# jematy/SAHS-Deformable-Nerf

Measured on AMD Instinct MI355X. Metric: rendered rays/sec (coarse64+fine128, 8x256 MLP), higher is better.
Workload: dtype f32

## Files before the change

### sahs-deformable-nerf_amd/csrc/f32_pipe.hpp

```cpp
#pragma once
#include <hip/hip_runtime.h>
#include "sahs_common.hpp"
#include "sahs_layout.hpp"

namespace SAHS_NS {

constexpr int F32_THREADS = 512;
constexpr int F32_PTS_PER_WAVE = 16;
constexpr int F32_PTS_PER_WG = (F32_THREADS / WAVE) * F32_PTS_PER_WAVE;
constexpr int DBG_STRIDE = 56;
constexpr int LDS_BUF_FLOATS = CHUNK_FLOATS_MAX;
constexpr int LDS_BIAS_OFF = 2 * LDS_BUF_FLOATS;
constexpr int LDS_FLOATS = LDS_BIAS_OFF + ((BIAS_FLOATS + 3) / 4) * 4;
static_assert(LDS_FLOATS * 4 <= 160 * 1024, "LDS budget");

typedef __attribute__((address_space(3))) void *lds_ptr_t;
typedef const __attribute__((address_space(1))) void *gbl_ptr_t;
typedef const __attribute__((address_space(3))) float *lds_cfloat;
typedef const __attribute__((address_space(3))) f32x4 *lds_cf4;

constexpr int LDS_STASH_OFF = LDS_BIAS_OFF + ((BIAS_FLOATS + 3) / 4) * 4;
constexpr int STASH_FLOATS = 8;
constexpr int LDS_TOTAL_FLOATS = LDS_STASH_OFF + F32_PTS_PER_WG * STASH_FLOATS;
static_assert(LDS_TOTAL_FLOATS * 4 <= 160 * 1024, "LDS budget");
constexpr int PIECE_FLOATS = F32_THREADS * 4;
constexpr int MAX_PIECES = LDS_BUF_FLOATS / PIECE_FLOATS;
constexpr int A_AHEAD = 3;

struct Ctx {
    const float *stream;
    float *lds;
    int buf;
    int lane, q, wave;
    uint32_t off;
    uint32_t wrap_at, wrap_to;
    const f32x4 *nx_src; f32x4 *nx_dst;
    lds_cfloat bias_lane;

    __device__ __forceinline__ void begin_chunk(int next_floats)
    {
        if (off >= wrap_at) off = wrap_to;
        nx_src = reinterpret_cast<const f32x4 *>(stream + off) + lane;
        nx_dst = reinterpret_cast<f32x4 *>(lds + (buf ^ 1) * LDS_BUF_FLOATS);
        off += (uint32_t)next_floats;
    }
    __device__ __forceinline__ void issue_piece(int p)
    {
        const int base = p * F32_THREADS + wave * WAVE;
        __builtin_amdgcn_global_load_lds((gbl_ptr_t)(nx_src + base), (lds_ptr_t)(nx_dst + base), 16, 0, 0);
    }
    template <int N = 0>
    __device__ __forceinline__ void end_chunk()
    {
        if constexpr (N == 0) {
            __syncthreads();
        } else {
            asm volatile("s_waitcnt vmcnt(%0) lgkmcnt(0)\n\ts_barrier" ::"n"(N) : "memory");
        }
        buf ^= 1;
    }
    __device__ __forceinline__ const f32x4 *cur() const { return reinterpret_cast<const f32x4 *>(lds + buf * LDS_BUF_FLOATS); }
    __device__ __forceinline__ void refresh()
    {
        uint32_t a = (uint32_t)(uintptr_t)((__attribute__((address_space(3))) char *)lds) + (LDS_BIAS_OFF + 4 * q) * 4;
        asm volatile("" : "+v"(a));
        bias_lane = (lds_cfloat)(uintptr_t)a;
    }
    __device__ __forceinline__ f32x4 bias4(int off_) const { return *reinterpret_cast<lds_cf4>(bias_lane + off_); }
};

__device__ __forceinline__ f32x4 act4(f32x4 v, float slope)
{
    f32x4 o;
#pragma unroll
    for (int r = 0; r < 4; ++r) o[r] = fmaxf(v[r], v[r] * slope);
    return o;
}

constexpr int stores_behind_last_piece(int STEPS, int PAIR, int KB, int next_floats, int per_tile)
{
    const int npieces = (next_floats + PIECE_FLOATS - 1) / PIECE_FLOATS;
    const int pstep = (STEPS / 2 >= npieces) ? (STEPS / 2) / npieces : 1;
    if (per_tile == 0 || npieces > (STEPS + pstep - 1) / pstep) return 0;
    int n = 0;
    for (int s = (npieces - 1) * pstep; s < STEPS; ++s)
        if ((s % (PAIR * KB)) / PAIR == KB - 1) n += per_tile;
    return n > 48 ? 48 : n;
}

template <int KB0, int KB1, int NT, int NEXT, class EP>
__device__ __forceinline__ void dense_ep(Ctx &cx, const f32x4 *in0, const f32x4 *in1, f32x4 *out, EP &ep)
{
    constexpr int KB = KB0 + KB1;
    constexpr int G = pick_G(KB, NT);
    constexpr int NCH = NT / G;
    constexpr int PAIR = (G >= 2) ? 2 : 1;
    constexpr int STEPS = G * KB;
    constexpr int N_MID = stores_behind_last_piece(STEPS, PAIR, KB, G * KB * 256, EP::kStores), N_LAST = stores_behind_last_piece(STEPS, PAIR, KB, NEXT, EP::kStores);
#pragma unroll
    for (int c = 0; c < NCH; ++c) {
        const int nfl = (c + 1 < NCH) ? G * KB * 256 : NEXT;
        const int npieces = (nfl + PIECE_FLOATS - 1) / PIECE_FLOATS;
        const int pstep = (STEPS / 2 >= npieces) ? (STEPS / 2) / npieces : 1;
        cx.begin_chunk(nfl);
        const f32x4 *A = cx.cur() + cx.lane;
        auto frag = [&](int s) { const int pp = s / (PAIR * KB), r = s % (PAIR * KB); return ((pp * PAIR + r % PAIR) * KB + r / PAIR) * 64; };
        f32x4 a[A_AHEAD];
#pragma unroll
        for (int s = 0; s < A_AHEAD && s < STEPS; ++s) a[s] = A[frag(s)];
        f32x4 acc[PAIR];
#pragma unroll
        for (int s = 0; s < STEPS; ++s) {
            const int pp = s / (PAIR * KB), r = s % (PAIR * KB), m = r % PAIR, b = r / PAIR;
            const int t = c * G + pp * PAIR + m;
            if (b == 0) acc[m] = ep.first(cx, out, t);
            if (s % pstep == 0 && s / pstep < npieces) {
                cx.issue_piece(s / pstep);
                if (EP::kStores > 0 && s / pstep == npieces - 1) __builtin_amdgcn_sched_barrier(0);
            }
            const f32x4 x = (b < KB0) ? in0[b] : in1[b - KB0];
            const f32x4 w = a[s % A_AHEAD];
#pragma unroll
            for (int k = 0; k < 4; ++k) acc[m] = __builtin_amdgcn_mfma_f32_16x16x4f32(w[k], x[k], acc[m], 0, 0, 0);
            if (s + A_AHEAD < STEPS) a[s % A_AHEAD] = A[frag(s + A_AHEAD)];
            if (b == KB - 1) ep.template done<NT>(acc[m], out, t);
        }
#pragma unroll
        for (int pc = (STEPS + pstep - 1) / pstep; pc < MAX_PIECES; ++pc)
            if (pc < npieces) cx.issue_piece(pc);
        if (c + 1 < NCH) cx.template end_chunk<N_MID>();
        else cx.template end_chunk<N_LAST>();
    }
}

template <bool HAS_SAVE>
struct FwdEp {
    static constexpr int kStores = HAS_SAVE ? 1 : 0;
    int bias_off; bool accum; float slope;
    float *save;
    uint32_t *bsave;
    uint32_t sgn;
    __device__ __forceinline__ f32x4 first(const Ctx &cx, const f32x4 *out, int t) const { return accum ? out[t] : cx.bias4(bias_off + 16 * t); }
    template <int NT> __device__ __forceinline__ void done(const f32x4 &acc, f32x4 *out, int t)
    {
        f32x4 o = act4(acc, slope);
        asm volatile("" : "+v"(o));
        out[t] = o;
        if constexpr (HAS_SAVE) *reinterpret_cast<f32x4 *>(save + 16 * t) = o;
        if (bsave != nullptr) {
            uint32_t nib = 0u;
#pragma unroll
            for (int r = 0; r < 4; ++r) nib |= (o[r] > 0.0f) ? (1u << r) : 0u;
            if ((t & 1) == 0 && t + 1 < NT) sgn = nib;
            else reinterpret_cast<unsigned char *>(bsave)[t >> 1] = (unsigned char)((t & 1) ? (sgn | (nib << 4)) : nib);
        }
    }
};

template <int KB0, int KB1, int NT, int NEXT>
__device__ __forceinline__ void dense(Ctx &cx, const f32x4 *in0, const f32x4 *in1, f32x4 *out, int bias_off, bool accum, float slope)
{
    FwdEp<false> ep{bias_off, accum, slope, nullptr, nullptr, 0u};
    dense_ep<KB0, KB1, NT, NEXT>(cx, in0, in1, out, ep);
}
template <bool SAVING, int KB0, int KB1, int NT, int NEXT>
__device__ __forceinline__ void dense_sv(Ctx &cx, const f32x4 *in0, const f32x4 *in1, f32x4 *out, int bias_off, bool accum, float slope,
                                         float *save, uint32_t *bsave = nullptr)
{
    FwdEp<SAVING> ep{bias_off, accum, slope, save, SAVING ? bsave : nullptr, 0u};
    dense_ep<KB0, KB1, NT, NEXT>(cx, in0, in1, out, ep);
}

}
```

### sahs-deformable-nerf_amd/csrc/field_f32.hip

```cpp
#include <hip/hip_runtime.h>
#include "sahs_common.hpp"
#include "sahs_launchers.hpp"
#include "sahs_layout.hpp"
#include "f32_pipe.hpp"

namespace SAHS_NS {


struct RevArg { float p, lo; };
__device__ __forceinline__ RevArg rev_arg(float x)
{
    const float C_HI = 0.15915494f;
    const float C_LO = 6.4206382e-09f;
    RevArg r;
    r.p = x * C_HI;
    r.lo = fmaf(x, C_LO, fmaf(x, C_HI, -r.p));
    return r;
}
__device__ __forceinline__ float sin_octave(RevArg u, float scale, int fn)
{
    const float P = u.p * scale, Lo = u.lo * scale;
    const float f = (P - rintf(P)) + Lo;
    const float qf = rintf(4.0f * f);
    const float th = fmaf(qf, -0.25f, f) * 6.2831855f;
    const float z = th * th;
    const float sp = fmaf(th * z, fmaf(fmaf(-1.9515295891e-4f, z, 8.3321608736e-3f), z, -1.6666654611e-1f), th);
    const float cp = fmaf(z * z, fmaf(fmaf(2.443315711809948e-5f, z, -1.388731625493765e-3f), z, 4.166664568298827e-2f), fmaf(z, -0.5f, 1.0f));
    const int m = ((int)qf + fn) & 3;
    const float v = (m & 1) ? cp : sp;
    return (m & 2) ? -v : v;
}

template <int D, int L, int NB, int INC = 1>
__device__ __forceinline__ void pe_blocks(const float *v, int q, f32x4 *out)
{
    constexpr int D0 = INC ? D : 0;
    constexpr int W = D0 + 2 * D * L;
    const float v0 = v[0], v1 = v[D > 1 ? 1 : 0], v2 = v[D > 2 ? 2 : 0];
    const RevArg u0 = rev_arg(v0), u1 = rev_arg(v1), u2 = rev_arg(v2);
#pragma unroll
    for (int b = 0; b < NB; ++b)
#pragma unroll
        for (int r = 0; r < 4; ++r) {
            const int f = 16 * b + 4 * q + r;
            float val = 0.0f;
            if (f < D0) {
                val = (f == 0) ? v0 : ((f == 1) ? v1 : v2);
            } else if (f < W) {
                const int g = f - D0;
                const int k = g / (2 * D), rem = g % (2 * D);
                const int fn = rem / D, ax = rem % D;
                RevArg a;
                a.p = (ax == 0) ? u0.p : ((ax == 1) ? u1.p : u2.p);
                a.lo = (ax == 0) ? u0.lo : ((ax == 1) ? u1.lo : u2.lo);
                val = sin_octave(a, (float)(1 << k), fn);
            }
            out[b][r] = val;
        }
}

__device__ __forceinline__ void grid_blocks(const float *__restrict__ grid, float x, float y, float z, int q, f32x4 *out)
{
    const float R1 = (float)(G_RES - 1);
    const float ix = ((x + 1.0f) / 2.0f) * R1, iy = ((y + 1.0f) / 2.0f) * R1, iz = ((z + 1.0f) / 2.0f) * R1;
    const float fx = floorf(ix), fy = floorf(iy), fz = floorf(iz);
    const float x1 = fx + 1.0f, y1 = fy + 1.0f, z1 = fz + 1.0f;
    const float wx[2] = {x1 - ix, ix - fx}, wy[2] = {y1 - iy, iy - fy}, wz[2] = {z1 - iz, iz - fz};
    const bool ok = fx >= -1.0f && fx <= (float)G_RES && fy >= -1.0f && fy <= (float)G_RES && fz >= -1.0f && fz <= (float)G_RES;
    const int xi = ok ? (int)fx : -2, yi = ok ? (int)fy : -2, zi = ok ? (int)fz : -2;
    out[0] = f32x4{0.0f, 0.0f, 0.0f, 0.0f};
    out[1] = f32x4{0.0f, 0.0f, 0.0f, 0.0f};
#pragma unroll
    for (int n = 0; n < 8; ++n) {
        const int cx = xi + (n & 1), cy = yi + ((n >> 1) & 1), cz = zi + (n >> 2);
        const bool inb = cx >= 0 && cx < G_RES && cy >= 0 && cy < G_RES && cz >= 0 && cz < G_RES;
        const float wt = (wx[n & 1] * wy[(n >> 1) & 1]) * wz[n >> 2];
        const long vox = inb ? (((long)cz * G_RES + cy) * G_RES + cx) : 0;
        const f32x4 *g = reinterpret_cast<const f32x4 *>(grid + vox * D_GRID) + q;
        const f32x4 g0 = g[0], g1 = g[4];
        const float we = inb ? wt : 0.0f;
#pragma unroll
        for (int r = 0; r < 4; ++r) { out[0][r] = out[0][r] + g0[r] * we; out[1][r] = out[1][r] + g1[r] * we; }
    }
}

__device__ __forceinline__ void trunk_encodings(const float *stash, int q, f32x4 *enc)
{
    const float xw[3] = {stash[0], stash[1], stash[2]}, amb[2] = {stash[3], stash[4]};
    pe_blocks<3, L_XYZ, KB_XYZ>(xw, q, enc);
#if SAHS_MODEL != 2
    pe_blocks<AMB_DIM, L_AMB, KB_AMB, AMB_INC>(amb, q, enc + KB_XYZ);
#else
    (void)amb;
#endif
}

#define CHF(id) (kProg.layer[id].G * kProg.layer[id].KB * 256)

enum { FIELD_ALL = 0, FIELD_DEFORM = 1, FIELD_RADIANCE = 2, FIELD_ALL_FUSED = 6, FIELD_RADIANCE_FUSED = 7 };
constexpr int SPARSE_RING = 512;
static_assert(SPARSE_RING >= 255 + 128 && SPARSE_RING % 128 == 0, "a ring holds the carried count plus one tile");
__host__ __device__ constexpr long sparse_ring_slots(long tiles) { return tiles * F32_PTS_PER_WG < SPARSE_RING ? tiles * F32_PTS_PER_WG : SPARSE_RING; }
__host__ __device__ constexpr long sparse_ring_base(long ntiles, long grid, long g)
{
    const long tlo = ntiles / grid, rem = ntiles % grid;
    return g * sparse_ring_slots(tlo) + (g < rem ? g : rem) * (sparse_ring_slots(tlo + 1) - sparse_ring_slots(tlo));
}
constexpr int LDS_RING_FLOATS = 16;
struct SparseArgs {
    const float *noise;
    unsigned int *count;
    f32x4 *hdr;
    f32x4 *feat;
    unsigned int cap;
    int has_bg;
};
constexpr long SPARSE_HEAD_BYTES = 256, SPARSE_RECORD_BYTES = 16 + 16 * 16 * 4;
template <bool SAVE, int MODE>
__global__ void __launch_bounds__(F32_THREADS, 2)
field_forward_f32_kernel(const float *__restrict__ packed, const float *__restrict__ frame, int level, long P, int S,
                         const float *__restrict__ rays, int ray_stride, const float *__restrict__ zvals,
                         float *__restrict__ raw, float *__restrict__ dbg, float *__restrict__ actbuf,
                         float *__restrict__ xw, int xw_row, int xw_col0, const int *__restrict__ src, uint32_t *__restrict__ bits, SparseArgs sp)
{
#if SAHS_MODEL == 2
    static_assert(MODE == FIELD_ALL || MODE == FIELD_ALL_FUSED, "this model has no deformation nets to split off");
#endif
    constexpr bool FUSED = MODE == FIELD_ALL_FUSED || MODE == FIELD_RADIANCE_FUSED;
    constexpr bool XW_IN = MODE == FIELD_RADIANCE || MODE == FIELD_RADIANCE_FUSED;
    static_assert(!(SAVE && FUSED), "the sparse branches are an inference path");
    extern __shared__ __attribute__((aligned(16))) float lds[];
    Ctx cx;
    cx.stream = packed + PACK_STREAM_OFF + (long)level * STREAM_FLOATS;
    cx.lds = lds;
    cx.buf = 1;
    cx.lane = threadIdx.x & 63;
    cx.q = cx.lane >> 4;
    cx.wave = __builtin_amdgcn_readfirstlane(threadIdx.x >> 6);
    constexpr const Layer *Ly = kProg.layer;
    constexpr int L_START = XW_IN ? L_T0 : L_FIRST;
    cx.wrap_to = (uint32_t)Ly[L_START].stream_off;
    cx.wrap_at = (MODE == FIELD_DEFORM) ? (uint32_t)Ly[L_T0].stream_off : (FUSED ? (uint32_t)Ly[L_D0B].stream_off : (uint32_t)STREAM_FLOATS);
    cx.off = cx.wrap_to;
    const float *grid = packed + PACK_GRID_OFF;

    {
        const float *bsrc = frame + FRAME_BIAS_OFF + level * BIAS_FLOATS;
        for (int i = threadIdx.x; i < BIAS_FLOATS; i += F32_THREADS) lds[LDS_BIAS_OFF + i] = bsrc[i];
        cx.begin_chunk(CHF(L_START));
#pragma unroll
        for (int pc = 0; pc < (CHF(L_START) + PIECE_FLOATS - 1) / PIECE_FLOATS; ++pc) cx.issue_piece(pc);
        cx.end_chunk();
    }

    const long ntiles = (P + F32_PTS_PER_WG - 1) / F32_PTS_PER_WG;
    constexpr bool XW_AHEAD = MODE == FIELD_RADIANCE_FUSED;
    f32x4 nx_a = f32x4{0.0f, 0.0f, 0.0f, 0.0f};
    float nx_w1 = 0.0f;
    int nx_src = 0;
    uint32_t r_cnt = 0u, r_head = 0u, r_total = 0u, r_cap = 0u, r_base = 0u;
    uint32_t r_it = 0u, r_tiles = 0u;
    if constexpr (FUSED) {
        r_tiles = (uint32_t)__builtin_amdgcn_readfirstlane((int)(ntiles / gridDim.x + ((long)blockIdx.x < ntiles % gridDim.x ? 1 : 0)));
        r_cap = (uint32_t)sparse_ring_slots(r_tiles);
        r_base = (uint32_t)__builtin_amdgcn_readfirstlane((int)sparse_ring_base(ntiles, gridDim.x, blockIdx.x));
    }
    const uint32_t r_rows = FUSED ? (uint32_t)__builtin_amdgcn_readfirstlane((int)(ntiles / gridDim.x)) : 0u;
    auto fused_tile = [&](uint32_t k) -> long {
        const uint32_t col = k < r_rows ? (blockIdx.x + 61u * k) % gridDim.x : blockIdx.x;
        return (long)k * gridDim.x + col;
    };
    for (long tile_it = blockIdx.x; FUSED || tile_it < ntiles; tile_it += gridDim.x, ++r_it) {
        const long tile = FUSED ? fused_tile(r_it) : tile_it;
        bool has_tile = true, do_branch = false;
        uint32_t b_valid = 0u;
        if constexpr (FUSED) {
            has_tile = r_it < r_tiles;
            do_branch = has_tile ? r_cnt >= (uint32_t)F32_PTS_PER_WG : r_cnt > 0u;
            if (!has_tile && !do_branch) break;
            b_valid = r_cnt < (uint32_t)F32_PTS_PER_WG ? r_cnt : (uint32_t)F32_PTS_PER_WG;
            if (has_tile) {
                cx.wrap_at = do_branch ? (uint32_t)STREAM_FLOATS : (uint32_t)Ly[L_D0B].stream_off;
            } else {
                cx.off = (uint32_t)Ly[L_D0B].stream_off;
                cx.wrap_at = (uint32_t)STREAM_FLOATS;
                cx.begin_chunk(CHF(L_D0B));
#pragma unroll
                for (int pc = 0; pc < (CHF(L_D0B) + PIECE_FLOATS - 1) / PIECE_FLOATS; ++pc) cx.issue_piece(pc);
                cx.end_chunk();
            }
        }
        cx.refresh();
        int q_tile = cx.q;
        if constexpr (FUSED) { asm volatile("" : "+s"(cx.off)); asm volatile("" : "+v"(q_tile)); }
        const int q = q_tile;
        const long p_raw = tile * F32_PTS_PER_WG + cx.wave * F32_PTS_PER_WAVE + (cx.lane & 15);
        const long p = p_raw < P ? p_raw : P - 1;
        float *stash = lds + LDS_STASH_OFF + (cx.wave * F32_PTS_PER_WAVE + (cx.lane & 15)) * STASH_FLOATS;
        const bool dump = MODE == FIELD_ALL && dbg != nullptr && q == 0 && p_raw < P;
        float *dsl = dbg + p * DBG_STRIDE;
        const bool sv_on = SAVE && p_raw < P;
        long Psv = P;
        if constexpr (SAVE) asm volatile("" : "+s"(Psv));
#define SVP(c, w) (actbuf + (long)(c) * Psv + p * (long)(w) + 4 * q)
#define SV(c, w) SVP(c, w)
        const bool sb_on = sv_on && bits != nullptr;
        uint32_t *const bits_r = bits + (MODE == FIELD_ALL ? (long)sbits::BD_WORDS * Psv : 0L);
        const uint32_t sb_lane = (uint32_t)(p * 4 + q);
#define SBD(b, w) (sb_on ? bits + (long)(b) * Psv + sb_lane * (uint32_t)((w) >= 128 ? (w) / 128 : 1) : nullptr)
#define SBR(b, w) (sb_on ? bits_r + (long)(b) * Psv + sb_lane * (uint32_t)((w) >= 128 ? (w) / 128 : 1) : nullptr)
        float x[3] = {0.0f, 0.0f, 0.0f};
        long smp = p;
        if constexpr (!XW_IN) {
            if (!FUSED || has_tile) {
            const float *rp = rays + (p / S) * ray_stride;
            const float z = zvals[p];
#pragma unroll
            for (int i = 0; i < 3; ++i) x[i] = rp[i] + rp[3 + i] * z;
            }
        } else if constexpr (XW_AHEAD) {
            if (q == 0 && has_tile) {
                if (r_it == 0u) {
                    const float *row = xw + ((p / S) * (long)xw_row + src[p]) * 8;
                    nx_a = *reinterpret_cast<const f32x4 *>(row);
                    nx_w1 = row[4];
                }
                stash[0] = nx_a[0]; stash[1] = nx_a[1]; stash[2] = nx_a[2]; stash[3] = nx_a[3]; stash[4] = nx_w1;
            }
        } else if (q == 0) {
            const float *row = xw + ((p / S) * (long)xw_row + src[p]) * 8;
            const f32x4 a = *reinterpret_cast<const f32x4 *>(row);
            stash[0] = a[0]; stash[1] = a[1]; stash[2] = a[2]; stash[3] = a[3]; stash[4] = row[4];
            if (sv_on) { float *d = SVP(act::XW, 16); d[0] = a[0]; d[1] = a[1]; d[2] = a[2]; }
        }
        const bool has_next = XW_AHEAD && r_it + 1u < r_tiles;
        const long pn_raw = fused_tile(r_it + 1u) * F32_PTS_PER_WG + cx.wave * F32_PTS_PER_WAVE + (cx.lane & 15);
        const long p_next = pn_raw < P ? pn_raw : P - 1;
        if constexpr (XW_AHEAD) {
            if (has_next && q == 0) nx_src = src[p_next];
        }
        f32x4 b_hdr = f32x4{0.0f, 0.0f, 0.0f, 0.0f};
        uint32_t b_slot = 0u;
        if constexpr (FUSED) {
            if (do_branch) {
                const uint32_t j = (uint32_t)(cx.wave * F32_PTS_PER_WAVE + (cx.lane & 15));
                b_slot = r_base + r_head + (j < b_valid ? j : b_valid - 1u);
                if (!has_tile) b_hdr = sp.hdr[b_slot];
            }
        }
        if constexpr (!XW_IN) {
        if (!FUSED || has_tile) {
#if SAHS_MODEL == 2
        if (q == 0) {
            stash[0] = x[0]; stash[1] = x[1]; stash[2] = x[2]; stash[3] = 0.0f; stash[4] = 0.0f;
            if (sv_on) { float *d = SVP(act::XW, 16); d[0] = x[0]; d[1] = x[1]; d[2] = x[2]; }
        }
#else
        f32x4 pe_x[KB_XYZ];
        {
            pe_blocks<3, L_XYZ, KB_XYZ>(x, q, pe_x);
            if (sv_on) {
#pragma unroll
                for (int b = 0; b < KB_XYZ; ++b) *reinterpret_cast<f32x4 *>(SVP(act::E, 16 * KB_XYZ) + 16 * b) = pe_x[b];
            }
        }
        {
            f32x4 h[8], hn[8];
            dense_sv<SAVE, KB_XYZ, 0, 8, CHF(L_W1)>(cx, pe_x, nullptr, h, Ly[L_W0].bias_off, false, 0.0f, SV(act::WH, 128), SBD(sbits::BD_WH + 4 * (0), 128));
            constexpr int W_ROLLED = (CHF(L_W4B) == CHF(L_W2)) ? 3 : 2;
#pragma unroll 1
            for (int l = 0; l < W_ROLLED; ++l) {
                dense_sv<SAVE, 8, 0, 8, CHF(L_W2)>(cx, h, nullptr, hn, Ly[L_W1].bias_off + 128 * l, false, 0.0f, SV(act::WH + 128 * (l + 1), 128), SBD(sbits::BD_WH + 4 * ((l + 1)), 128));
#pragma unroll
                for (int i = 0; i < 8; ++i) h[i] = hn[i];
            }
            if (W_ROLLED == 2) {
                dense_sv<SAVE, 8, 0, 8, CHF(L_W4B)>(cx, h, nullptr, hn, Ly[L_W3].bias_off, false, 0.0f, SV(act::WH + 128 * 3, 128), SBD(sbits::BD_WH + 4 * (3), 128));
#pragma unroll
                for (int i = 0; i < 8; ++i) h[i] = hn[i];
            }
            dense<KB_XYZ, 0, 8, CHF(L_W4A)>(cx, pe_x, nullptr, hn, Ly[L_W4B].bias_off, false, 1.0f);
// ... 51 lines not shown
        f32x4 feat[16];
        if (!FUSED || has_tile) {
            f32x4 h[16];
            if constexpr (FUSED) {
                constexpr bool ENC_ONCE = MODE == FIELD_RADIANCE_FUSED;
                f32x4 in_tr[KB_XYZ + KB_AMB];
                auto build_enc = [&]() { trunk_encodings(stash, q, in_tr); };
                build_enc();
                dense<KB_XYZ, KB_AMB, 16, CHF(L_T1)>(cx, in_tr, in_tr + KB_XYZ, h, Ly[L_T0].bias_off, false, 0.01f);
                if (do_branch) b_hdr = sp.hdr[b_slot];
                dense<16, 0, 16, CHF(L_T2)>(cx, h, nullptr, feat, Ly[L_T1].bias_off, false, 0.01f);
#pragma unroll
                for (int i = 0; i < 16; ++i) h[i] = feat[i];
                dense<16, 0, 16, CHF(L_T3B)>(cx, h, nullptr, feat, Ly[L_T2].bias_off, false, 0.01f);
#pragma unroll
                for (int i = 0; i < 16; ++i) h[i] = feat[i];
                if constexpr (XW_AHEAD) {
                    if (has_next && q == 0) {
                        const float *row = xw + ((p_next / S) * (long)xw_row + nx_src) * 8;
                        nx_a = *reinterpret_cast<const f32x4 *>(row);
                        nx_w1 = row[4];
                    }
                }
                if constexpr (!ENC_ONCE) build_enc();
                dense<KB_XYZ, KB_AMB, 16, CHF(L_T3A)>(cx, in_tr, in_tr + KB_XYZ, feat, Ly[L_T3B].bias_off, false, 1.0f);
            } else {
            {
                f32x4 in_tr[KB_XYZ + KB_AMB];
                trunk_encodings(stash, q, in_tr);
                if (sv_on) {
#pragma unroll
                    for (int b = 0; b < KB_XYZ + KB_AMB; ++b)
                        *reinterpret_cast<f32x4 *>(b < KB_XYZ ? SVP(act::PEX, 16 * KB_XYZ) + 16 * b : SVP(act::PEW, 16 * KB_AMB) + 16 * (b - KB_XYZ)) = in_tr[b];
                }
                dense_sv<SAVE, KB_XYZ, KB_AMB, 16, CHF(L_T1)>(cx, in_tr, in_tr + KB_XYZ, h, Ly[L_T0].bias_off, false, 0.01f, SV(act::T, 256), SBR(sbits::BR_T + 8 * (0), 256));
            }
            if (dump) dsl[5] = h[0][0];
            dense_sv<SAVE, 16, 0, 16, CHF(L_T2)>(cx, h, nullptr, feat, Ly[L_T1].bias_off, false, 0.01f, SV(act::T + 256, 256), SBR(sbits::BR_T + 8 * (1), 256));
            if (dump) dsl[6] = feat[0][0];
#pragma unroll
            for (int i = 0; i < 16; ++i) h[i] = feat[i];
            dense_sv<SAVE, 16, 0, 16, CHF(L_T3B)>(cx, h, nullptr, feat, Ly[L_T2].bias_off, false, 0.01f, SV(act::T + 512, 256), SBR(sbits::BR_T + 8 * (2), 256));
            if (dump) dsl[7] = feat[0][0];
#pragma unroll
            for (int i = 0; i < 16; ++i) h[i] = feat[i];
            {
                f32x4 in_tr[KB_XYZ + KB_AMB];
                trunk_encodings(stash, q, in_tr);
                dense<KB_XYZ, KB_AMB, 16, CHF(L_T3A)>(cx, in_tr, in_tr + KB_XYZ, feat, Ly[L_T3B].bias_off, false, 1.0f);
            }
            }
#if SAHS_MODEL == 0
            dense_sv<SAVE, 16, 0, 16, CHF(L_T4)>(cx, h, nullptr, feat, 0, true, 0.01f, SV(act::T + 768, 256), SBR(sbits::BR_T + 8 * (3), 256));
#else
            dense_sv<SAVE, 16, 0, 16, CHF(L_FEAT)>(cx, h, nullptr, feat, 0, true, 0.01f, SV(act::T + 768, 256), SBR(sbits::BR_T + 8 * (3), 256));
#endif
            if (dump) dsl[8] = feat[0][0];
#pragma unroll
            for (int i = 0; i < 16; ++i) h[i] = feat[i];
#if SAHS_MODEL == 0
#pragma unroll 1
            for (int l = 4; l <= 7; ++l) {
                dense_sv<SAVE, 16, 0, 16, CHF(L_T5)>(cx, h, nullptr, feat, Ly[L_T4].bias_off + 256 * (l - 4), false, 0.01f, SV(act::T + 256 * l, 256), SBR(sbits::BR_T + 8 * (l), 256));
                if (dump) dsl[5 + l] = feat[0][0];
#pragma unroll
                for (int i = 0; i < 16; ++i) h[i] = feat[i];
            }
#endif
            dense_sv<SAVE, 16, 0, 16, CHF(L_ALPHA)>(cx, h, nullptr, feat, Ly[L_FEAT].bias_off, false, 1.0f, SV(act::FEAT, 256));
            if (dump) dsl[13] = feat[0][0];
        }
        if (!FUSED || has_tile) {
            if (FUSED && !do_branch) dense<16, 0, 1, CHF(L_START)>(cx, feat, nullptr, fin, Ly[L_ALPHA].bias_off, false, 1.0f);
            else dense<16, 0, 1, CHF(L_D0B)>(cx, feat, nullptr, fin, Ly[L_ALPHA].bias_off, false, 1.0f);
        }
        if constexpr (FUSED) {
            if (has_tile) {
                if (p_raw < P) *reinterpret_cast<f32x4 *>(raw + p * D_RAW + 4 * q) = fin[0];
                const long ray = p / S;
                const bool last = (p - ray * S) == S - 1;
                const float sg = fin[0][3] + (sp.noise != nullptr ? sp.noise[p] : 0.0f);
                const bool live = q == 3 && p_raw < P && (last ? sp.has_bg == 0 : sg > 0.0f);
                const uint32_t mask = (uint32_t)(__ballot(live) >> 48);
                uint32_t *cnts = reinterpret_cast<uint32_t *>(lds + LDS_TOTAL_FLOATS);
                if (cx.lane == 0) cnts[cx.wave] = (uint32_t)__popc(mask);
                __syncthreads();
                uint32_t before = 0u, all = 0u;
#pragma unroll
                for (int w = 0; w < F32_THREADS / WAVE; ++w) {
                    const uint32_t c = cnts[w];
                    all += c;
                    before += w < cx.wave ? c : 0u;
                }
                before = (uint32_t)__builtin_amdgcn_readfirstlane((int)before);
                all = (uint32_t)__builtin_amdgcn_readfirstlane((int)all);
                uint32_t tail = r_head + r_cnt;
                if (tail >= r_cap) tail -= r_cap;
                const int j = cx.lane & 15;
                if ((mask >> j) & 1u) {
                    uint32_t idx = tail + before + (uint32_t)__popc(mask & ((1u << j) - 1u));
                    if (idx >= r_cap) idx -= r_cap;
                    const uint32_t slot = r_base + idx;
                    f32x4 *rec = sp.feat + (long)(slot >> 4) * (16 * 64) + q * 16 + (slot & 15u);
#pragma unroll
                    for (int b = 0; b < 16; ++b) rec[b * 64] = feat[b];
                    if (q == 0) sp.hdr[slot] = f32x4{stash[0], stash[1], stash[2], __int_as_float((int)p)};
                }
                r_cnt += all;
                r_total += all;
            }
            if (!do_branch) continue;
            smp = __float_as_int(b_hdr[3]);
            __builtin_amdgcn_wave_barrier();
            if (q == 0) { stash[0] = b_hdr[0]; stash[1] = b_hdr[1]; stash[2] = b_hdr[2]; }
            __builtin_amdgcn_wave_barrier();
            fin[0] = *reinterpret_cast<const f32x4 *>(raw + smp * D_RAW + 4 * q);
            const f32x4 *rec = sp.feat + (long)(b_slot >> 4) * (16 * 64) + q * 16 + (b_slot & 15u);
#pragma unroll
            for (int b = 0; b < 16; ++b) feat[b] = rec[b * 64];
            r_cnt -= b_valid;
            r_head += (uint32_t)F32_PTS_PER_WG;
            if (r_head >= r_cap) r_head -= r_cap;
        }
        if (dbg != nullptr && p_raw < P) *reinterpret_cast<f32x4 *>(dsl + 24 + 4 * q) = fin[0];
        {
            f32x4 in_d[4];
            {
                const float *rp = rays + (smp / S) * ray_stride;
                const float rd[3] = {rp[3], rp[4], rp[5]};
                pe_blocks<3, 4, 2>(rd, q, in_d);
                grid_blocks(grid, stash[0], stash[1], stash[2], q, in_d + 2);
                if (sv_on) {
#pragma unroll
                    for (int b = 0; b < 4; ++b) *reinterpret_cast<f32x4 *>(b < 2 ? SVP(act::DIR, 32) + 16 * b : SVP(act::GRID, 32) + 16 * (b - 2)) = in_d[b];
                }
            }
            if (dbg != nullptr && p_raw < P) {
                float *d = dbg + P * DBG_STRIDE + p * 32;
                *reinterpret_cast<f32x4 *>(d + 4 * q) = in_d[2];
                *reinterpret_cast<f32x4 *>(d + 16 + 4 * q) = in_d[3];
            }
            f32x4 c[8], cn[8];
            dense<2, 2, 8, CHF(L_D0A)>(cx, in_d, in_d + 2, c, Ly[L_D0B].bias_off, false, 1.0f);
            dense_sv<SAVE, 16, 0, 8, CHF(L_D1)>(cx, feat, nullptr, c, 0, true, 0.01f, SV(act::C, 128), SBR(sbits::BR_C + 4 * (0), 128));
            if (dump) dsl[14] = c[0][0];
#pragma unroll 1
            for (int l = 0; l < 2; ++l) {
                dense_sv<SAVE, 8, 0, 8, CHF(L_D2)>(cx, c, nullptr, cn, Ly[L_D1].bias_off + 128 * l, false, 0.01f, SV(act::C + 128 * (l + 1), 128), SBR(sbits::BR_C + 4 * ((l + 1)), 128));
#pragma unroll
                for (int i = 0; i < 8; ++i) c[i] = cn[i];
            }
            dense_sv<SAVE, 8, 0, 8, CHF(L_RGB)>(cx, c, nullptr, cn, Ly[L_D3].bias_off, false, 0.01f, SV(act::C + 384, 128), SBR(sbits::BR_C + 4 * (3), 128));
            if (dump) dsl[15] = cn[0][0];
            dense<8, 0, 1, CHF(L_S0)>(cx, cn, nullptr, fin, 0, true, 1.0f);
            if (dbg != nullptr && p_raw < P) *reinterpret_cast<f32x4 *>(dsl + 40 + 4 * q) = fin[0];
        }
        {
            f32x4 s[8], sn[8];
            dense_sv<SAVE, 16, 0, 8, CHF(L_S1)>(cx, feat, nullptr, s, Ly[L_S0].bias_off, false, 0.01f, SV(act::S, 128), SBR(sbits::BR_S + 4 * (0), 128));
            if (dump) dsl[16] = s[0][0];
#pragma unroll 1
            for (int l = 0; l < 2; ++l) {
                dense_sv<SAVE, 8, 0, 8, CHF(L_S2)>(cx, s, nullptr, sn, Ly[L_S1].bias_off + 128 * l, false, 0.01f, SV(act::S + 128 * (l + 1), 128), SBR(sbits::BR_S + 4 * ((l + 1)), 128));
#pragma unroll
                for (int i = 0; i < 8; ++i) s[i] = sn[i];
            }
            dense_sv<SAVE, 8, 0, 8, CHF(L_SEG)>(cx, s, nullptr, sn, Ly[L_S3].bias_off, false, 0.01f, SV(act::S + 384, 128), SBR(sbits::BR_S + 4 * (3), 128));
            if (dump) dsl[17] = sn[0][0];
            dense<8, 0, 1, CHF(L_START)>(cx, sn, nullptr, fin, 0, true, 1.0f);
        }
        if (FUSED ? (uint32_t)(cx.wave * F32_PTS_PER_WAVE + (cx.lane & 15)) < b_valid : p_raw < P)
            *reinterpret_cast<f32x4 *>(raw + smp * D_RAW + 4 * q) = fin[0];
    }
    if constexpr (FUSED) {
        if (threadIdx.x == 0) {
            if (r_total != 0u) atomicAdd(sp.count, r_total);
            if (blockIdx.x == 0) sp.count[1] = 1u;
        }
    }
}

}

using namespace SAHS_NS;

template <bool SAVE, int MODE>
static int launch_field(const FieldLaunch &L, SparseArgs sp = SparseArgs{})
{
    const size_t lds_bytes = (size_t)(LDS_TOTAL_FLOATS + ((MODE == FIELD_ALL_FUSED || MODE == FIELD_RADIANCE_FUSED) ? LDS_RING_FLOATS : 0)) * sizeof(float);
    return sahs_launch_persistent<field_forward_f32_kernel<SAVE, MODE>>((L.P + F32_PTS_PER_WG - 1) / F32_PTS_PER_WG, L.num_cu, F32_THREADS, lds_bytes, L.stream,
                                                                        L.packed, L.frame, L.level, L.P, L.S, L.rays, L.ray_stride, L.zvals, L.raw, L.dbg,
                                                                        L.actbuf, L.xw, L.xw_row, L.xw_col0, L.src, L.bits, sp);
}

extern "C" int SAHS_SYM(sahs_field_f32_launch)(const FieldLaunch *in, int mode)
{
    if (in->P <= 0) return 0;
    FieldLaunch L = sahs_field_mode_block(*in, mode);
    const bool save = L.actbuf != nullptr;
    if (!save) L.bits = nullptr;
#if SAHS_MODEL == 2
    if (mode != FIELD_ALL || (!save && L.xw != nullptr)) return -3;
#endif
    switch (mode) {
    case FIELD_ALL: return save ? launch_field<true, FIELD_ALL>(L) : launch_field<false, FIELD_ALL>(L);
#if SAHS_MODEL != 2
    case FIELD_DEFORM: return save ? launch_field<true, FIELD_DEFORM>(L) : launch_field<false, FIELD_DEFORM>(L);
    case FIELD_RADIANCE: return save ? launch_field<true, FIELD_RADIANCE>(L) : launch_field<false, FIELD_RADIANCE>(L);
#endif
    default: return -2;
    }
}

extern "C" long SAHS_SYM(sahs_field_f32_sparse_ws_bytes)(long cap) { return SPARSE_HEAD_BYTES + cap * SPARSE_RECORD_BYTES; }
extern "C" long SAHS_SYM(sahs_field_f32_sparse_ring_slots)(long P, int num_cu)
{
    if (P <= 0 || num_cu < 1) return 0;
    const long ntiles = (P + F32_PTS_PER_WG - 1) / F32_PTS_PER_WG, grid = ntiles < num_cu ? ntiles : num_cu;
    return sparse_ring_base(ntiles, grid, grid);
}
extern "C" int SAHS_SYM(sahs_field_f32_sparse_launch)(const FieldLaunch *in, int stage, const float *noise, int has_bg, void *ws, long cap)
{
    if (in->P <= 0) return 0;
    if (ws == nullptr || cap % F32_PTS_PER_WG != 0 || cap > (1L << 30)) return -4;
    if (cap < SAHS_SYM(sahs_field_f32_sparse_ring_slots)(in->P, in->num_cu)) return -4;
    char *base = static_cast<char *>(ws);
    SparseArgs sp{noise, reinterpret_cast<unsigned int *>(base), reinterpret_cast<f32x4 *>(base + SPARSE_HEAD_BYTES),
                  reinterpret_cast<f32x4 *>(base + SPARSE_HEAD_BYTES + cap * 16), (unsigned int)cap, has_bg};
    FieldLaunch L = sahs_field_mode_block(*in, stage == 0 ? FIELD_ALL : FIELD_RADIANCE);
    L.dbg = L.actbuf = nullptr;
    L.bits = nullptr;
    if (stage == 0) return launch_field<false, FIELD_ALL_FUSED>(L, sp);
#if SAHS_MODEL != 2
    if (stage == 1) return launch_field<false, FIELD_RADIANCE_FUSED>(L, sp);
#endif
    return -2;
}

extern "C" int SAHS_SYM(sahs_layout_act_part_words)(int part) { return part == 1 ? act::XW + 16 : (part == 2 ? act::STRIDE - act::XW : act::STRIDE); }
extern "C" int SAHS_SYM(sahs_layout_act_part_col0)(int part) { return part == 2 ? act::XW : 0; }
extern "C" int SAHS_SYM(sahs_layout_bits_part_words)(int part) { return part == 1 ? sbits::BD_WORDS : (part == 2 ? sbits::BR_WORDS : sbits::BD_WORDS + sbits::BR_WORDS); }
```

### sahs-deformable-nerf_amd/csrc/sahs_layout.hpp

```cpp
#pragma once
#include <cstdint>
#include "sahs_model.hpp"

namespace SAHS_NS {

#if SAHS_MODEL == 0
constexpr int L_XYZ = 10, AMB_DIM = 2, L_AMB = 4, AMB_INC = 1, TR_LAYERS = 8;
constexpr bool TRUNK_SEES_POSE = true, HAS_AUDIONET = true, USE_DEFORM = true;
#elif SAHS_MODEL == 1
constexpr int L_XYZ = 15, AMB_DIM = 1, L_AMB = 15, AMB_INC = 0, TR_LAYERS = 4;
constexpr bool TRUNK_SEES_POSE = false, HAS_AUDIONET = false, USE_DEFORM = true;
#else
constexpr int L_XYZ = 10, AMB_DIM = 0, L_AMB = 0, AMB_INC = 0, TR_LAYERS = 4;
constexpr bool TRUNK_SEES_POSE = false, HAS_AUDIONET = false, USE_DEFORM = false;
#endif
constexpr int D_XYZ = 3 + 6 * L_XYZ;
constexpr int D_AMB = AMB_INC * AMB_DIM + 2 * AMB_DIM * L_AMB;
constexpr int KB_XYZ = (D_XYZ + 15) / 16, KB_AMB = (D_AMB + 15) / 16;
constexpr int D_DIR = 27, D_POSE = 36, D_DRV = 76, D_GRID = 32, G_RES = 32;
constexpr int WARP_H = 128, HYP_H = 64, TR_H = 256, BR_H = 128, N_SEG = 12, D_RAW = 16;
constexpr int D_TR_CONST = TRUNK_SEES_POSE ? D_POSE : D_DRV;
constexpr int TR_CONST_WHICH = TRUNK_SEES_POSE ? 1 : 0;
constexpr int D_DEF_IN = D_XYZ + D_DRV + D_POSE;
constexpr int D_TR_IN = D_XYZ + D_AMB + D_TR_CONST;
// ... 16 lines not shown
{
    FlatOffsets f{};
    long p = 0;
    f.grid = p; p += GRID_FLOATS;
    if (USE_DEFORM) {
        for (int i = 0; i < 6; ++i) {
            int in = (i == 0) ? D_DEF_IN : (i == 4 ? WARP_H + D_DEF_IN : WARP_H);
            f.warp_w[i] = p; p += (long)WARP_H * in; f.warp_b[i] = p; p += WARP_H;
        }
        f.warp_fw = p; p += 3 * WARP_H; f.warp_fb = p; p += 3;
        for (int i = 0; i < 6; ++i) {
            int in = (i == 0) ? D_DEF_IN : (i == 4 ? HYP_H + D_DEF_IN : HYP_H);
            f.hyp_w[i] = p; p += (long)HYP_H * in; f.hyp_b[i] = p; p += HYP_H;
        }
        f.hyp_fw = p; p += AMB_DIM * HYP_H; f.hyp_fb = p; p += AMB_DIM;
    }
    for (int l = 0; l < 2; ++l) {
        for (int i = 0; i < TR_LAYERS; ++i) {
            int in = (i == 0) ? D_TR_IN : (i == 3 ? TR_H + D_TR_IN : TR_H);
            f.lvl[l].xyz_w[i] = p; p += (long)TR_H * in; f.lvl[l].xyz_b[i] = p; p += TR_H;
        }
        f.lvl[l].feat_w = p; p += TR_H * TR_H; f.lvl[l].feat_b = p; p += TR_H;
        f.lvl[l].alpha_w = p; p += TR_H; f.lvl[l].alpha_b = p; p += 1;
        for (int i = 0; i < 4; ++i) {
            int in = (i == 0) ? D_DIR_IN : BR_H;
            f.lvl[l].dir_w[i] = p; p += (long)BR_H * in; f.lvl[l].dir_b[i] = p; p += BR_H;
        }
        f.lvl[l].rgb_w = p; p += 3 * BR_H; f.lvl[l].rgb_b = p; p += 3;
        for (int i = 0; i < 4; ++i) {
            int in = (i == 0) ? TR_H : BR_H;
            f.lvl[l].seg_w[i] = p; p += (long)BR_H * in; f.lvl[l].seg_b[i] = p; p += BR_H;
        }
        f.lvl[l].segout_w = p; p += N_SEG * BR_H; f.lvl[l].segout_b = p; p += N_SEG;
    }
    if (HAS_AUDIONET) {
        constexpr int cin[4] = {29, 32, 32, 64}, cout[4] = {32, 32, 64, 64};
        for (int i = 0; i < 4; ++i) { f.conv_w[i] = p; p += (long)cout[i] * cin[i] * 3; f.conv_b[i] = p; p += cout[i]; }
        f.fc_w[0] = p; p += 64 * 64; f.fc_b[0] = p; p += 64;
        f.fc_w[1] = p; p += D_DRV * 64; f.fc_b[1] = p; p += D_DRV;
    }
    f.total = p;
    return f;
}
constexpr FlatOffsets kFlat = make_flat_offsets();
static_assert(kFlat.total == (SAHS_MODEL == 0 ? 2775633 : (SAHS_MODEL == 1 ? 2311140 : 2066976)),
              "flat parameter count must match the reference state_dict");

struct Seg { int blocks; int src_col; int valid; };
struct Fold { int src_col; int count; int which; };
enum LayerId {
#if SAHS_MODEL != 2
    L_W0, L_W1, L_W2, L_W3, L_W4B, L_W4A, L_W5, L_WF,
    L_H0, L_H1, L_H2, L_H3, L_H4B, L_H4A, L_H5, L_HF,
#endif
    L_T0, L_T1, L_T2, L_T3B, L_T3A,
#if SAHS_MODEL == 0
    L_T4, L_T5, L_T6, L_T7,
#endif
    L_FEAT, L_ALPHA,
    L_D0B, L_D0A, L_D1, L_D2, L_D3, L_RGB,
    L_S0, L_S1, L_S2, L_S3, L_SEG,
    NUM_LAYERS,
    L_FIRST = 0
};
struct Layer {
    long w_off[2];
    long b_off[2];
    int src_ld;
    int src_rows;
    int row_shift;
    int NT;
    int KB;
    int G;
    int nseg; Seg seg[2];
    int nfold; Fold fold[2];
    int has_bias;
    int bias_off;
    int bias_shared;
    long stream_off;
    int first_chunk;
};

constexpr int CHUNK_FLOATS_MAX = 8192;
constexpr int pick_G(int KB, int NT)
{
    int g = CHUNK_FLOATS_MAX / (KB * 256);
    if (g > NT) g = NT;
    while (NT % g) --g;
    return g;
}

struct Program {
    Layer layer[NUM_LAYERS];
    int bias_floats;
    long stream_floats;
    int num_chunks;
};

struct Src { long w0, w1, b0, b1; int ld, rows; };

constexpr Layer mk(Src s, int has_bias, int shift, int NT, Seg s0, Seg s1 = {0, 0, 0}, Fold f0 = {0, 0, 0}, Fold f1 = {0, 0, 0})
{
    Layer L{};
    L.w_off[0] = s.w0; L.w_off[1] = s.w1; L.b_off[0] = s.b0; L.b_off[1] = s.b1;
    L.src_ld = s.ld; L.src_rows = s.rows; L.row_shift = shift; L.NT = NT; L.has_bias = has_bias;
    L.seg[0] = s0; L.seg[1] = s1;
    L.nseg = 1 + (s1.blocks > 0);
    L.KB = s0.blocks + s1.blocks;
    L.fold[0] = f0; L.fold[1] = f1;
    L.nfold = (f0.count > 0) + (f1.count > 0);
    L.G = pick_G(L.KB, NT);
    return L;
}

constexpr Program make_program()
{
    Program P{};
    const FlatOffsets &f = kFlat;
    Layer *L = P.layer;
#if SAHS_MODEL != 2
    auto warp = [&](int i, int ld) { return Src{f.warp_w[i], f.warp_w[i], f.warp_b[i], f.warp_b[i], ld, WARP_H}; };
    auto hyp = [&](int i, int ld) { return Src{f.hyp_w[i], f.hyp_w[i], f.hyp_b[i], f.hyp_b[i], ld, HYP_H}; };
    L[L_W0] = mk(warp(0, D_DEF_IN), 1, 0, 8, {KB_XYZ, 0, D_XYZ}, {0, 0, 0}, {D_XYZ, D_DRV, 0}, {D_XYZ + D_DRV, D_POSE, 1});
    L[L_W1] = mk(warp(1, WARP_H), 1, 0, 8, {8, 0, 128});
    L[L_W2] = mk(warp(2, WARP_H), 1, 0, 8, {8, 0, 128});
    L[L_W3] = mk(warp(3, WARP_H), 1, 0, 8, {8, 0, 128});
    L[L_W4B] = mk(warp(4, WARP_H + D_DEF_IN), 1, 0, 8, {KB_XYZ, WARP_H, D_XYZ}, {0, 0, 0}, {WARP_H + D_XYZ, D_DRV, 0},
                  {WARP_H + D_XYZ + D_DRV, D_POSE, 1});
    L[L_W4A] = mk(warp(4, WARP_H + D_DEF_IN), 0, 0, 8, {8, 0, 128});
    L[L_W5] = mk(warp(5, WARP_H), 1, 0, 8, {8, 0, 128});
    L[L_WF] = mk(Src{f.warp_fw, f.warp_fw, f.warp_fb, f.warp_fb, WARP_H, 3}, 1, 0, 1, {8, 0, 128});
    L[L_H0] = mk(hyp(0, D_DEF_IN), 1, 0, 4, {KB_XYZ, 0, D_XYZ}, {0, 0, 0}, {D_XYZ, D_DRV, 0}, {D_XYZ + D_DRV, D_POSE, 1});
    L[L_H1] = mk(hyp(1, HYP_H), 1, 0, 4, {4, 0, 64});
    L[L_H2] = mk(hyp(2, HYP_H), 1, 0, 4, {4, 0, 64});
    L[L_H3] = mk(hyp(3, HYP_H), 1, 0, 4, {4, 0, 64});
    L[L_H4B] = mk(hyp(4, HYP_H + D_DEF_IN), 1, 0, 4, {KB_XYZ, HYP_H, D_XYZ}, {0, 0, 0}, {HYP_H + D_XYZ, D_DRV, 0},
                  {HYP_H + D_XYZ + D_DRV, D_POSE, 1});
    L[L_H4A] = mk(hyp(4, HYP_H + D_DEF_IN), 0, 0, 4, {4, 0, 64});
    L[L_H5] = mk(hyp(5, HYP_H), 1, 0, 4, {4, 0, 64});
    L[L_HF] = mk(Src{f.hyp_fw, f.hyp_fw, f.hyp_fb, f.hyp_fb, HYP_H, AMB_DIM}, 1, 0, 1, {4, 0, 64});
#endif
    const FlatOffsets::Lvl &c = f.lvl[0], &n = f.lvl[1];
    auto tr = [&](int i, int ld) { return Src{c.xyz_w[i], n.xyz_w[i], c.xyz_b[i], n.xyz_b[i], ld, TR_H}; };
    L[L_T0] = mk(tr(0, D_TR_IN), 1, 0, 16, {KB_XYZ, 0, D_XYZ}, {KB_AMB, D_XYZ, D_AMB}, {D_XYZ + D_AMB, D_TR_CONST, TR_CONST_WHICH});
    L[L_T1] = mk(tr(1, TR_H), 1, 0, 16, {16, 0, 256});
    L[L_T2] = mk(tr(2, TR_H), 1, 0, 16, {16, 0, 256});
    L[L_T3B] = mk(tr(3, TR_H + D_TR_IN), 1, 0, 16, {KB_XYZ, TR_H, D_XYZ}, {KB_AMB, TR_H + D_XYZ, D_AMB},
                  {TR_H + D_XYZ + D_AMB, D_TR_CONST, TR_CONST_WHICH});
    L[L_T3A] = mk(tr(3, TR_H + D_TR_IN), 0, 0, 16, {16, 0, 256});
#if SAHS_MODEL == 0
    for (int i = 4; i < 8; ++i) L[L_T4 + (i - 4)] = mk(tr(i, TR_H), 1, 0, 16, {16, 0, 256});
#endif
    L[L_FEAT] = mk(Src{c.feat_w, n.feat_w, c.feat_b, n.feat_b, TR_H, TR_H}, 1, 0, 16, {16, 0, 256});
    L[L_ALPHA] = mk(Src{c.alpha_w, n.alpha_w, c.alpha_b, n.alpha_b, TR_H, 1}, 1, 15, 1, {16, 0, 256});
    auto dir = [&](int i, int ld) { return Src{c.dir_w[i], n.dir_w[i], c.dir_b[i], n.dir_b[i], ld, BR_H}; };
    L[L_D0B] = mk(dir(0, D_DIR_IN), 1, 0, 8, {2, 256, 27}, {2, 283, 32});
    L[L_D0A] = mk(dir(0, D_DIR_IN), 0, 0, 8, {16, 0, 256});
    for (int i = 1; i < 4; ++i) L[L_D0A + i] = mk(dir(i, BR_H), 1, 0, 8, {8, 0, 128});
    L[L_RGB] = mk(Src{c.rgb_w, n.rgb_w, c.rgb_b, n.rgb_b, BR_H, 3}, 1, 0, 1, {8, 0, 128});
    auto sg = [&](int i, int ld) { return Src{c.seg_w[i], n.seg_w[i], c.seg_b[i], n.seg_b[i], ld, BR_H}; };
    L[L_S0] = mk(sg(0, TR_H), 1, 0, 8, {16, 0, 256});
    for (int i = 1; i < 4; ++i) L[L_S0 + i] = mk(sg(i, BR_H), 1, 0, 8, {8, 0, 128});
    L[L_SEG] = mk(Src{c.segout_w, n.segout_w, c.segout_b, n.segout_b, BR_H, N_SEG}, 1, 3, 1, {8, 0, 128});

    int boff = 0; long soff = 0; int chunk = 0;
    int final_bias = -1;
    for (int i = 0; i < NUM_LAYERS; ++i) {
        const bool fin = (i == L_ALPHA || i == L_RGB || i == L_SEG);
        if (fin) {
            if (final_bias < 0) { final_bias = boff; boff += 16; }
            L[i].bias_off = final_bias; L[i].bias_shared = 1;
        } else if (L[i].has_bias) {
            L[i].bias_off = boff; boff += L[i].NT * 16;
// ... 164 lines not shown
```

Measured before the change: 458,700.

## Double LDS weight chunk capacity for inference field kernel with deeper prefetch

Templates the LDS weight-streaming context on chunk capacity so the non-saving (inference) field kernel uses twice-as-large double-buffered weight chunks. More output tiles are processed per chunk, which cuts the number of barriers and chunk switches per layer, and the A-fragment lookahead goes from three to four with a scheduling barrier pinning each step. The trade is much higher LDS use per workgroup, which can lower occupancy, plus more register pressure from the deeper prefetch.

```diff
diff --git a/sahs-deformable-nerf_amd/csrc/f32_pipe.hpp b/sahs-deformable-nerf_amd/csrc/f32_pipe.hpp
--- a/sahs-deformable-nerf_amd/csrc/f32_pipe.hpp
+++ b/sahs-deformable-nerf_amd/csrc/f32_pipe.hpp
@@ -9,25 +9,32 @@
 constexpr int F32_PTS_PER_WAVE = 16;
 constexpr int F32_PTS_PER_WG = (F32_THREADS / WAVE) * F32_PTS_PER_WAVE;
 constexpr int DBG_STRIDE = 56;
-constexpr int LDS_BUF_FLOATS = CHUNK_FLOATS_MAX;
-constexpr int LDS_BIAS_OFF = 2 * LDS_BUF_FLOATS;
-constexpr int LDS_FLOATS = LDS_BIAS_OFF + ((BIAS_FLOATS + 3) / 4) * 4;
-static_assert(LDS_FLOATS * 4 <= 160 * 1024, "LDS budget");
 
 typedef __attribute__((address_space(3))) void *lds_ptr_t;
 typedef const __attribute__((address_space(1))) void *gbl_ptr_t;
 typedef const __attribute__((address_space(3))) float *lds_cfloat;
 typedef const __attribute__((address_space(3))) f32x4 *lds_cf4;
 
-constexpr int LDS_STASH_OFF = LDS_BIAS_OFF + ((BIAS_FLOATS + 3) / 4) * 4;
 constexpr int STASH_FLOATS = 8;
-constexpr int LDS_TOTAL_FLOATS = LDS_STASH_OFF + F32_PTS_PER_WG * STASH_FLOATS;
-static_assert(LDS_TOTAL_FLOATS * 4 <= 160 * 1024, "LDS budget");
 constexpr int PIECE_FLOATS = F32_THREADS * 4;
-constexpr int MAX_PIECES = LDS_BUF_FLOATS / PIECE_FLOATS;
-constexpr int A_AHEAD = 3;
+constexpr int CHUNK_FLOATS_WIDE = 2 * CHUNK_FLOATS_MAX;
+constexpr int a_ahead(int cap) { return cap > CHUNK_FLOATS_MAX ? 4 : 3; }
+constexpr bool a_pinned(int cap) { return cap > CHUNK_FLOATS_MAX; }
+template <int CAP>
+struct LdsMap {
+    static constexpr int BUF_FLOATS = CAP;
+    static constexpr int BIAS_OFF = 2 * BUF_FLOATS;
+    static constexpr int STASH_OFF = BIAS_OFF + ((BIAS_FLOATS + 3) / 4) * 4;
+    static constexpr int TOTAL_FLOATS = STASH_OFF + F32_PTS_PER_WG * STASH_FLOATS;
+    static constexpr int MAX_PIECES = BUF_FLOATS / PIECE_FLOATS;
+    static_assert(BUF_FLOATS % PIECE_FLOATS == 0, "a buffer is whole DMA pieces");
+    static_assert(TOTAL_FLOATS * 4 <= 160 * 1024, "LDS budget");
+};
+constexpr int LDS_BUF_FLOATS = LdsMap<CHUNK_FLOATS_MAX>::BUF_FLOATS;
+constexpr int MAX_PIECES = LdsMap<CHUNK_FLOATS_MAX>::MAX_PIECES;
 
-struct Ctx {
+template <int CAP>
+struct CtxT {
     const float *stream;
     float *lds;
     int buf;
@@ -41,7 +48,7 @@
     {
         if (off >= wrap_at) off = wrap_to;
         nx_src = reinterpret_cast<const f32x4 *>(stream + off) + lane;
-        nx_dst = reinterpret_cast<f32x4 *>(lds + (buf ^ 1) * LDS_BUF_FLOATS);
+        nx_dst = reinterpret_cast<f32x4 *>(lds + (buf ^ 1) * CAP);
         off += (uint32_t)next_floats;
     }
     __device__ __forceinline__ void issue_piece(int p)
@@ -59,15 +66,16 @@
         }
         buf ^= 1;
     }
-    __device__ __forceinline__ const f32x4 *cur() const { return reinterpret_cast<const f32x4 *>(lds + buf * LDS_BUF_FLOATS); }
+    __device__ __forceinline__ const f32x4 *cur() const { return reinterpret_cast<const f32x4 *>(lds + buf * CAP); }
     __device__ __forceinline__ void refresh()
     {
-        uint32_t a = (uint32_t)(uintptr_t)((__attribute__((address_space(3))) char *)lds) + (LDS_BIAS_OFF + 4 * q) * 4;
+        uint32_t a = (uint32_t)(uintptr_t)((__attribute__((address_space(3))) char *)lds) + (LdsMap<CAP>::BIAS_OFF + 4 * q) * 4;
         asm volatile("" : "+v"(a));
         bias_lane = (lds_cfloat)(uintptr_t)a;
     }
     __device__ __forceinline__ f32x4 bias4(int off_) const { return *reinterpret_cast<lds_cf4>(bias_lane + off_); }
 };
+typedef CtxT<CHUNK_FLOATS_MAX> Ctx;
 
 __device__ __forceinline__ f32x4 act4(f32x4 v, float slope)
 {
@@ -88,14 +96,15 @@
     return n > 48 ? 48 : n;
 }
 
-template <int KB0, int KB1, int NT, int NEXT, class EP>
-__device__ __forceinline__ void dense_ep(Ctx &cx, const f32x4 *in0, const f32x4 *in1, f32x4 *out, EP &ep)
+template <int KB0, int KB1, int NT, int NEXT, class EP, int CAP>
+__device__ __forceinline__ void dense_ep(CtxT<CAP> &cx, const f32x4 *in0, const f32x4 *in1, f32x4 *out, EP &ep)
 {
     constexpr int KB = KB0 + KB1;
-    constexpr int G = pick_G(KB, NT);
+    constexpr int G = pick_G(KB, NT, CAP);
     constexpr int NCH = NT / G;
     constexpr int PAIR = (G >= 2) ? 2 : 1;
     constexpr int STEPS = G * KB;
+    constexpr int A_AHEAD = a_ahead(CAP);
     constexpr int N_MID = stores_behind_last_piece(STEPS, PAIR, KB, G * KB * 256, EP::kStores), N_LAST = stores_behind_last_piece(STEPS, PAIR, KB, NEXT, EP::kStores);
 #pragma unroll
     for (int c = 0; c < NCH; ++c) {
@@ -123,10 +132,11 @@
 #pragma unroll
             for (int k = 0; k < 4; ++k) acc[m] = __builtin_amdgcn_mfma_f32_16x16x4f32(w[k], x[k], acc[m], 0, 0, 0);
             if (s + A_AHEAD < STEPS) a[s % A_AHEAD] = A[frag(s + A_AHEAD)];
+            if constexpr (a_pinned(CAP)) __builtin_amdgcn_sched_barrier(0);
             if (b == KB - 1) ep.template done<NT>(acc[m], out, t);
         }
 #pragma unroll
-        for (int pc = (STEPS + pstep - 1) / pstep; pc < MAX_PIECES; ++pc)
+        for (int pc = (STEPS + pstep - 1) / pstep; pc < LdsMap<CAP>::MAX_PIECES; ++pc)
             if (pc < npieces) cx.issue_piece(pc);
         if (c + 1 < NCH) cx.template end_chunk<N_MID>();
         else cx.template end_chunk<N_LAST>();
@@ -140,7 +150,7 @@
     float *save;
     uint32_t *bsave;
     uint32_t sgn;
-    __device__ __forceinline__ f32x4 first(const Ctx &cx, const f32x4 *out, int t) const { return accum ? out[t] : cx.bias4(bias_off + 16 * t); }
+    template <class CX> __device__ __forceinline__ f32x4 first(const CX &cx, const f32x4 *out, int t) const { return accum ? out[t] : cx.bias4(bias_off + 16 * t); }
     template <int NT> __device__ __forceinline__ void done(const f32x4 &acc, f32x4 *out, int t)
     {
         f32x4 o = act4(acc, slope);
@@ -157,14 +167,14 @@
     }
 };
 
-template <int KB0, int KB1, int NT, int NEXT>
-__device__ __forceinline__ void dense(Ctx &cx, const f32x4 *in0, const f32x4 *in1, f32x4 *out, int bias_off, bool accum, float slope)
+template <int KB0, int KB1, int NT, int NEXT, int CAP>
+__device__ __forceinline__ void dense(CtxT<CAP> &cx, const f32x4 *in0, const f32x4 *in1, f32x4 *out, int bias_off, bool accum, float slope)
 {
     FwdEp<false> ep{bias_off, accum, slope, nullptr, nullptr, 0u};
     dense_ep<KB0, KB1, NT, NEXT>(cx, in0, in1, out, ep);
 }
-template <bool SAVING, int KB0, int KB1, int NT, int NEXT>
-__device__ __forceinline__ void dense_sv(Ctx &cx, const f32x4 *in0, const f32x4 *in1, f32x4 *out, int bias_off, bool accum, float slope,
+template <bool SAVING, int KB0, int KB1, int NT, int NEXT, int CAP>
+__device__ __forceinline__ void dense_sv(CtxT<CAP> &cx, const f32x4 *in0, const f32x4 *in1, f32x4 *out, int bias_off, bool accum, float slope,
                                          float *save, uint32_t *bsave = nullptr)
 {
     FwdEp<SAVING> ep{bias_off, accum, slope, save, SAVING ? bsave : nullptr, 0u};
diff --git a/sahs-deformable-nerf_amd/csrc/field_f32.hip b/sahs-deformable-nerf_amd/csrc/field_f32.hip
--- a/sahs-deformable-nerf_amd/csrc/field_f32.hip
+++ b/sahs-deformable-nerf_amd/csrc/field_f32.hip
@@ -95,7 +95,9 @@
 #endif
 }
 
-#define CHF(id) (kProg.layer[id].G * kProg.layer[id].KB * 256)
+constexpr int chunk_floats(int id, int cap) { return pick_G(kProg.layer[id].KB, kProg.layer[id].NT, cap) * kProg.layer[id].KB * 256; }
+#define CHF(id) chunk_floats(id, CAP)
+constexpr int field_chunk_cap(bool save) { return save ? CHUNK_FLOATS_MAX : CHUNK_FLOATS_WIDE; }
 
 enum { FIELD_ALL = 0, FIELD_DEFORM = 1, FIELD_RADIANCE = 2, FIELD_ALL_FUSED = 6, FIELD_RADIANCE_FUSED = 7 };
 constexpr int SPARSE_RING = 512;
@@ -107,6 +109,9 @@
     return g * sparse_ring_slots(tlo) + (g < rem ? g : rem) * (sparse_ring_slots(tlo + 1) - sparse_ring_slots(tlo));
 }
 constexpr int LDS_RING_FLOATS = 16;
+constexpr bool field_mode_fused(int mode) { return mode == 6 || mode == 7; }
+constexpr int field_lds_floats(bool save, int mode) { return (save ? LdsMap<field_chunk_cap(true)>::TOTAL_FLOATS : LdsMap<field_chunk_cap(false)>::TOTAL_FLOATS) + (field_mode_fused(mode) ? LDS_RING_FLOATS : 0); }
+static_assert(field_lds_floats(false, 7) * 4 <= 160 * 1024 && field_lds_floats(true, 0) * 4 <= 160 * 1024, "LDS budget of the largest instance of each cap");
 struct SparseArgs {
     const float *noise;
     unsigned int *count;
@@ -129,8 +134,10 @@
     constexpr bool FUSED = MODE == FIELD_ALL_FUSED || MODE == FIELD_RADIANCE_FUSED;
     constexpr bool XW_IN = MODE == FIELD_RADIANCE || MODE == FIELD_RADIANCE_FUSED;
     static_assert(!(SAVE && FUSED), "the sparse branches are an inference path");
+    constexpr int CAP = field_chunk_cap(SAVE);
+    typedef LdsMap<CAP> Lds;
     extern __shared__ __attribute__((aligned(16))) float lds[];
-    Ctx cx;
+    CtxT<CAP> cx;
     cx.stream = packed + PACK_STREAM_OFF + (long)level * STREAM_FLOATS;
     cx.lds = lds;
     cx.buf = 1;
@@ -146,7 +153,7 @@
 
     {
         const float *bsrc = frame + FRAME_BIAS_OFF + level * BIAS_FLOATS;
-        for (int i = threadIdx.x; i < BIAS_FLOATS; i += F32_THREADS) lds[LDS_BIAS_OFF + i] = bsrc[i];
+        for (int i = threadIdx.x; i < BIAS_FLOATS; i += F32_THREADS) lds[Lds::BIAS_OFF + i] = bsrc[i];
         cx.begin_chunk(CHF(L_START));
 #pragma unroll
         for (int pc = 0; pc < (CHF(L_START) + PIECE_FLOATS - 1) / PIECE_FLOATS; ++pc) cx.issue_piece(pc);
@@ -192,11 +199,11 @@
         }
         cx.refresh();
         int q_tile = cx.q;
-        if constexpr (FUSED) { asm volatile("" : "+s"(cx.off)); asm volatile("" : "+v"(q_tile)); }
+        if constexpr (FUSED || (!SAVE && TR_LAYERS == 4)) { asm volatile("" : "+s"(cx.off)); asm volatile("" : "+v"(q_tile)); }
         const int q = q_tile;
         const long p_raw = tile * F32_PTS_PER_WG + cx.wave * F32_PTS_PER_WAVE + (cx.lane & 15);
         const long p = p_raw < P ? p_raw : P - 1;
-        float *stash = lds + LDS_STASH_OFF + (cx.wave * F32_PTS_PER_WAVE + (cx.lane & 15)) * STASH_FLOATS;
+        float *stash = lds + Lds::STASH_OFF + (cx.wave * F32_PTS_PER_WAVE + (cx.lane & 15)) * STASH_FLOATS;
         const bool dump = MODE == FIELD_ALL && dbg != nullptr && q == 0 && p_raw < P;
         float *dsl = dbg + p * DBG_STRIDE;
         const bool sv_on = SAVE && p_raw < P;
@@ -414,7 +421,7 @@
                 const float sg = fin[0][3] + (sp.noise != nullptr ? sp.noise[p] : 0.0f);
                 const bool live = q == 3 && p_raw < P && (last ? sp.has_bg == 0 : sg > 0.0f);
                 const uint32_t mask = (uint32_t)(__ballot(live) >> 48);
-                uint32_t *cnts = reinterpret_cast<uint32_t *>(lds + LDS_TOTAL_FLOATS);
+                uint32_t *cnts = reinterpret_cast<uint32_t *>(lds + Lds::TOTAL_FLOATS);
                 if (cx.lane == 0) cnts[cx.wave] = (uint32_t)__popc(mask);
                 __syncthreads();
                 uint32_t before = 0u, all = 0u;
@@ -519,7 +526,7 @@
 template <bool SAVE, int MODE>
 static int launch_field(const FieldLaunch &L, SparseArgs sp = SparseArgs{})
 {
-    const size_t lds_bytes = (size_t)(LDS_TOTAL_FLOATS + ((MODE == FIELD_ALL_FUSED || MODE == FIELD_RADIANCE_FUSED) ? LDS_RING_FLOATS : 0)) * sizeof(float);
+    const size_t lds_bytes = (size_t)field_lds_floats(SAVE, MODE) * sizeof(float);
     return sahs_launch_persistent<field_forward_f32_kernel<SAVE, MODE>>((L.P + F32_PTS_PER_WG - 1) / F32_PTS_PER_WG, L.num_cu, F32_THREADS, lds_bytes, L.stream,
                                                                         L.packed, L.frame, L.level, L.P, L.S, L.rays, L.ray_stride, L.zvals, L.raw, L.dbg,
                                                                         L.actbuf, L.xw, L.xw_row, L.xw_col0, L.src, L.bits, sp);
diff --git a/sahs-deformable-nerf_amd/csrc/sahs_layout.hpp b/sahs-deformable-nerf_amd/csrc/sahs_layout.hpp
--- a/sahs-deformable-nerf_amd/csrc/sahs_layout.hpp
+++ b/sahs-deformable-nerf_amd/csrc/sahs_layout.hpp
@@ -122,13 +122,14 @@
 };
 
 constexpr int CHUNK_FLOATS_MAX = 8192;
-constexpr int pick_G(int KB, int NT)
-{
-    int g = CHUNK_FLOATS_MAX / (KB * 256);
+constexpr int pick_G(int KB, int NT, int cap)
+{
+    int g = cap / (KB * 256);
     if (g > NT) g = NT;
     while (NT % g) --g;
     return g;
 }
+constexpr int pick_G(int KB, int NT) { return pick_G(KB, NT, CHUNK_FLOATS_MAX); }
 
 struct Program {
     Layer layer[NUM_LAYERS];
```

Result: faster. 468,600 (median of 6 runs) (+2.2%).
